# richardbaihe/a3t

Hardware: AMD Instinct MI355X
Metric: mel-frames/sec (train) (higher is better)
Workload: dtype bf16; 1 GPU; VCTK A3T masked-mel train step: 6+6 Conformer blocks d=384 H=2 ff=1536(k3), B=32/GPU, T_mel=1000, T_phn=120, postnet 5x256x5, fwd+bwd+clip+Adam, dropout 0.2/0.2/0.2 + postnet 0.5 (recipe); global_batch=32, parallelism=dp1, params=100799808

## Files before the change

a3t_amd/_lib.py:

```python
import ctypes
import os
from ctypes import POINTER, c_char_p, c_float, c_int, c_int32, c_int64, c_void_p

import torch

HERE = os.path.dirname(os.path.abspath(__file__))
LIB_PATH = os.environ.get("A3T_LIB_PATH") or os.path.join(HERE, "lib", "liba3t_hip.so")

F32, BF16 = 0, 1
ACT_NONE, ACT_RELU, ACT_TANH, ACT_SWISH = 0, 1, 2, 3
ACC_STORE, ACC_ADD, ACC_ATOMIC, ACC_SOLE = 0, 1, 2, 3


class GemmDesc(ctypes.Structure):
    _fields_ = [
        ("A", c_void_p), ("B", c_void_p), ("C", c_void_p), ("bias", c_void_p), ("R", c_void_p), ("S", c_void_p),
        ("M", c_int32), ("N", c_int32), ("K", c_int32),
        ("a_rs", c_int64), ("a_cs", c_int64),
        ("b_rs", c_int64), ("b_cs", c_int64), ("b_ts", c_int64),
        ("c_rs", c_int64),
        ("batch", c_int32), ("batch_inner", c_int32),
        ("a_bs0", c_int64), ("a_bs1", c_int64), ("b_bs0", c_int64), ("b_bs1", c_int64),
        ("c_bs0", c_int64), ("c_bs1", c_int64),
        ("taps", c_int32), ("pad", c_int32), ("dil", c_int32), ("Tseq", c_int32), ("kshift", c_int32),
# ... 41 lines not shown
    "a3t_mask_fill": [_P, _P, _P, _P, c_int, c_int, c_int, _P],
    "a3t_embed_finish_fwd": [_P, _P, _P, _P, _P, _P, _P, c_int, c_int, c_int, c_int, c_float, c_float, ctypes.c_uint32,
                             _P, _P],
    "a3t_embed_finish_bwd": [_P, _P, _P, _P, _P, _P, _P, _P, c_int, c_int, c_int, c_int, c_int, c_int, c_float, c_float,
                             ctypes.c_uint32, _P],
    "a3t_scale": [_P, _P, c_int64, c_float, _P],
    "a3t_axpy": [_P, _P, c_int64, c_float, _P],
    "a3t_attn_bias_fold": [_P, c_int32, c_int32, _P, _P, _P, _P],
    "a3t_scale_dev": [_P, _P, c_int64, _P, _P],
    "a3t_slice_rows": [_P, _P, c_int, c_int, c_int, c_int, c_int, c_int, _P],
    "a3t_concat_rows": [_P, _P, _P, c_int, c_int, c_int, c_int, _P],
    "a3t_concat_rows_ragged": [_P, _P, _P, _P, _P, c_int, c_int, c_int, c_int, c_int64, c_int64, _P],
    "a3t_split_rows": [_P, _P, _P, c_int, c_int, c_int, c_int, _P],
    "a3t_cast_bf16": [_P, _P, c_int64, _P],
    "a3t_cast_bf16_conv_t": [_P, _P, _P, _P, c_int, c_int, c_int, c_int, _P],
    "a3t_split_bf16": [_P, _P, _P, c_int64, _P],
    "a3t_reflect_pad": [_P, _P, c_int, c_int, c_int, c_int, _P],
    "a3t_reflect_pad_ragged": [_P, _P, _P, c_int, c_int, c_int, c_int, _P],
    "a3t_stft_amp": [_P, _P, c_int64, c_int, c_int, _P],
    "a3t_logmel_finish": [_P, _P, c_int, c_int, c_int, _P],
    "a3t_mlm_loss": [_P, _P, _P, _P, _P, _P, _P, _P, c_int, c_int, c_int, c_float, _P],
    "a3t_mlm_loss_scratch_floats": [c_int],
    "a3t_sumsq": [_P, c_int64, _P, _P],
    "a3t_clip_adam": [_P, _P, _P, _P, _P, _P, c_int64, c_float, c_float, c_float, c_float, c_int, c_float, c_float,
                      _P],
    "a3t_clip_adam_noam": [_P, _P, _P, _P, _P, _P, c_int64, _P, c_float, c_float, c_float, c_float, c_float, c_float,
                           c_float, c_float, _P],
    "a3t_sgd_step": [_P, _P, c_int64, c_float, c_float, _P],
    "a3t_pwg_gate": [_P, _P, _P, c_int64, c_int, _P],
    "a3t_pwg_res_skip": [_P, _P, _P, c_int64, c_int, c_int, _P],
    "a3t_pwg_upsample": [_P, _P, _P, c_int64, c_int64, c_int, c_int, _P],
    "a3t_replicate_pad": [_P, _P, c_int64, c_int64, c_int, c_int, _P],
    "a3t_bias_act": [_P, _P, c_int64, c_int, c_int, c_float, _P],
    "a3t_replicate_pad_ragged": [_P, _P, _P, c_int64, c_int64, c_int, c_int, _P],
    "a3t_pwg_upsample_ragged": [_P, _P, _P, _P, c_int, c_int64, c_int64, c_int, c_int, _P],
    "a3t_zero_tail": [_P, _P, c_int, c_int64, c_int64, c_int, _P],
    "a3t_layernorm_fwd_ragged": [_P, _P, _P, _P, _P, _P, _P, c_int, c_int, c_int, c_float, _P],
    "a3t_glu_dwconv_fwd_ragged": [_P, _P, _P, _P, _P, _P, c_int, c_int, c_int, c_int, _P],
    "a3t_relpos_softmax_fwd_ragged": [_P, _P, c_int, _P, _P, c_int, c_int, c_int, c_int, c_int64, c_int64, c_int64, c_float,
                                      _P],
    "a3t_splice_spans": [_P, _P, _P, _P, _P, _P, c_int, c_int, c_int, c_int, _P],
    "a3t_pwg_block_ragged": [_P, _P, _P, _P, _P, _P, _P, _P, _P, c_int, c_int, c_int, c_int, _P],
# ... 75 lines not shown
```

a3t_amd/conformer.py:

```python
import math
import os
import zlib
from dataclasses import dataclass

import torch

from . import ops
from ._lib import ACC_ADD, ACC_ATOMIC, ACC_STORE, ACT_RELU, ACT_SWISH, BF16, F32
from .config import A3TConfig
from .params import ParamStore
from .schedule import StepSchedule


def legacy_pe_table(c: A3TConfig) -> torch.Tensor:
    d = c.adim
    position = torch.arange(c.max_len - 1, -1, -1.0, dtype=torch.float32).unsqueeze(1)
    div = torch.exp(torch.arange(0, d, 2, dtype=torch.float32) * -(math.log(10000.0) / d))
    pe = torch.zeros(c.max_len, d)
    pe[:, 0::2] = torch.sin(position * div)
    pe[:, 1::2] = torch.cos(position * div)
    return pe


def score_chunks(lengths, heads, max_score_elems):
# ... 27 lines not shown
    ffn_keep4: bool = True
    lin_dgrad_t: bool = True
    fuse_ln_dropout: bool = True

    @classmethod
    def from_env(cls, environ=os.environ):
        fa, ft = environ.get("A3T_FUSED_ATTN", "auto"), environ.get("A3T_FUSED_ATTN_TRAIN", "1")
        if fa not in ("auto", "fwd", "0"):
            raise ValueError(f"A3T_FUSED_ATTN={fa!r}: expected auto, fwd or 0 (the flash backward behind '1' left the library in "
                             "round 5, tools/experiments/attn_flash_backward.patch)")
        on = {f: environ.get("A3T_" + f.upper(), "1") != "0" for f in
              ("side_stream", "side2", "wgrad_group", "post_f32_first", "attn_bwd_ds", "attn_signed", "attn_dq_dual",
               "attn_dbd_view", "attn_dk_main", "ffn_8p", "ffn_keep4", "lin_dgrad_t")}
        return cls(side_depth=max(2, int(environ.get("A3T_SIDE_DEPTH", "48"))), fused_attn=fa,
                   fused_attn_train=0 if ft == "0" else 2 if ft == "2" else 1, **on)


class ConformerStack(StepSchedule):
    def __init__(self, cfg: A3TConfig, store: ParamStore, compute: str = "f32", training: bool = True,
                 dropout: bool = False, options: EngineOptions = None):
        self.opt = opt = options if options is not None else EngineOptions.from_env()
        super().__init__(store.device, opt.side_stream, opt.side2, opt.side_depth)
        self.c = cfg
        self.dropping = bool(dropout and training)
        self.step_seed = 0
        self.store = store
        self.bf16 = (compute == "bf16")
        self.adt = torch.bfloat16 if self.bf16 else torch.float32
        self.cmp = BF16 if self.bf16 else F32
        self.training = training
# ... 13 lines not shown
        self._fused_now = self._fused_train_now = False
        self.attn_path, self.block_dims = {}, {}
        self._need_grad = training
        self._mode_tag = None
        if self.bf16:
            for n, v in (("adim", cfg.adim), ("ff", cfg.ff), ("idim", cfg.idim), ("odim", cfg.odim),
                         ("dk", cfg.dk), ("postnet_chans", cfg.postnet_chans or 8)):
                if v % 8:
                    raise ValueError(f"compute='bf16' needs {n} % 8 == 0 (16-byte DMA granules), got {v}")
            self.flat16 = torch.zeros(store.total, dtype=torch.bfloat16, device=self.dev)
            self.p16 = {k: self.flat16[o:o + math.prod(s)].view(s) for k, (o, s) in store.offsets.items()}
        self._ffn_plans = {}
        self._lin_plans = {}
        self._wt = {}
        self._P_ahead, self._pos_ev = {}, None
        self._cast_ev = self._wt_ev = None
        dec = [o for k, (o, _) in store.offsets.items() if k.startswith("dec.")]
        self._cast_split = min(dec) if dec else 0

    def _drop(self, p, tag):
        if not self.dropping or p <= 0.0:
            return None
        h = (zlib.crc32(tag.encode()) ^ ((self.step_seed * 0x9E3779B1) & 0xFFFFFFFF)) & 0xFFFFFFFF
        h = ((h ^ (h >> 16)) * 0x85EBCA6B) & 0xFFFFFFFF
        h = ((h ^ (h >> 13)) * 0xC2B2AE35) & 0xFFFFFFFF
        return (float(p), (h ^ (h >> 16)) & 0xFFFFFFFF)

    def _gm(self, g, tag, p, bias_grad, bias_scale):
        dr = self._drop(p, tag)
        if dr is None:
            return (self._g16(g) if self.bf16 else g)
        gm = self.ws.get(self._t("tmp.gm"), tuple(g.shape), self.adt)
        if self._gm_ready == tag:
            self._gm_ready = None
            return gm
        ops.dropout_bwd_cast(g, gm, dr[0], dr[1], colsum=bias_grad, colsum_scale=bias_scale)
        return gm

    def W(self, name):
        return self.p16[name] if self.bf16 else self.store.p[name]

    def refresh_weights(self):
        self._cast_ev = self._wt_ev = None
        if not self.bf16:
            return
        split = self._cast_split if self.side is not None else 0
        flat, flat16 = self.store.flat, self.flat16
        wt = list(self._wt.values()) if self._need_grad else []

        def transposed():
            for src_off, dst_off, _, tflat, shp in wt:
                ops.cast_bf16_conv_t(flat, tflat, src_off, dst_off, *shp)
        if split <= 0:
            ops.cast_bf16(flat, flat16)
            transposed()
            return
        ops.cast_bf16(flat[:split], flat16[:split])
        self._cast_ev = self._side(lambda: ops.cast_bf16(flat[split:], flat16[split:]), want_event="cast")
        if wt:
            self._wt_ev = self._side(transposed, want_event="wt")

    def _wait_cast(self, which):
        ev = getattr(self, which, None)
# ... 512 lines not shown
```

a3t_amd/csrc/misc.hip:

```cpp
#include <hip/hip_runtime.h>
#include <math.h>
#include <stdint.h>
#include "../../include/a3t_hip.h"
#include "dtype_io.h"

static inline int nblocks(int64_t n, int cap = 4096) {
    int64_t b = (n + 255) / 256;
    return (int)(b > cap ? cap : (b < 1 ? 1 : b));
}
#define GRID_STRIDE(i, n) \
    for (int64_t i = (int64_t)blockIdx.x * blockDim.x + threadIdx.x; i < (n); i += (int64_t)gridDim.x * blockDim.x)

__global__ void mask_fill_kernel(const float* __restrict__ x, const uint8_t* __restrict__ m,
                                 const float* __restrict__ mf, void* __restrict__ y, int y_dt, int64_t n, int C) {
    GRID_STRIDE(i, n) {
        int64_t r = i / C;
        int c = (int)(i - r * C);
        stx(y, y_dt, i, m[r] ? mf[c] : x[i]);
    }
}
extern "C" int a3t_mask_fill(const float* speech, const uint8_t* masked, const float* mask_feature, void* out,
                             int out_dtype, int M, int C, void* stream) {
    int64_t n = (int64_t)M * C;
    hipLaunchKernelGGL(mask_fill_kernel, dim3(nblocks(n)), dim3(256), 0, (hipStream_t)stream, speech, masked,
// ... 155 lines not shown
    }
    __syncthreads();
    for (int r = ty; r < 32; r += 8) {
        const int c = c0 + r, n = n0 + tx;
        if (c < C && n < N) Wt[((int64_t)c * taps + (taps - 1 - t)) * N + n] = io_f2bf(tile[tx][r]);
    }
}
extern "C" int a3t_cast_bf16_conv_t(const float* src, void* dst, const int64_t* src_off, const int64_t* dst_off, int count, int N,
                                    int taps, int C, void* stream) {
    if (count <= 0 || N <= 0 || taps <= 0 || C <= 0) return A3T_EINVAL;
    if (taps > 65535 || count > 65535) return A3T_EINVAL;
    dim3 grid((unsigned)(((N + 31) / 32) * ((C + 31) / 32)), (unsigned)taps, (unsigned)count);
    hipLaunchKernelGGL(cast_conv_t_kernel, grid, dim3(256), 0, (hipStream_t)stream, src, (unsigned short*)dst, src_off, dst_off, N, taps, C);
    return (int)hipGetLastError();
}
__global__ void split_bf16_kernel(const float* __restrict__ x, unsigned short* __restrict__ hi, unsigned short* __restrict__ lo,
                                  int64_t n4) {
    GRID_STRIDE(i, n4) {
        const float4 v = ((const float4*)x)[i];
        uint2 h, l;
        h.x = io_pack2(v.x, v.y);
        h.y = io_pack2(v.z, v.w);
        l.x = io_pack2(v.x - io_bf2f(h.x & 0xffff), v.y - io_bf2f(h.x >> 16));
        l.y = io_pack2(v.z - io_bf2f(h.y & 0xffff), v.w - io_bf2f(h.y >> 16));
        ((uint2*)hi)[i] = h;
        ((uint2*)lo)[i] = l;
    }
}
extern "C" int a3t_split_bf16(const float* x, void* hi, void* lo, int64_t n, void* stream) {
    if (n % 4 || ((uintptr_t)x & 15) || ((uintptr_t)hi & 7) || ((uintptr_t)lo & 7)) return A3T_EINVAL;
// ... 221 lines not shown
    red[threadIdx.x] = s;
    __syncthreads();
    for (int o = 128; o > 0; o >>= 1) {
        if (threadIdx.x < o) red[threadIdx.x] += red[threadIdx.x + o];
        __syncthreads();
    }
    if (threadIdx.x == 0) partial[blockIdx.x] = red[0];
}
__device__ __forceinline__ void adam_elem(float& p, const float g, float& m, float& v, const float coef, const float b1, const float b2,
                                          const float step_size, const float bc2s, const float eps) {
    const float gi = g * coef;
    m = m * b1 + (1.f - b1) * gi;
    v = v * b2 + (1.f - b2) * gi * gi;
    p -= step_size * m / (sqrtf(v) / bc2s + eps);
}
__device__ __forceinline__ void adam_sweep(float* __restrict__ p, const float* __restrict__ g, float* __restrict__ m, float* __restrict__ v,
                                           const int64_t n, const float coef, const float b1, const float b2, const float step_size,
                                           const float bc2s, const float eps) {
    const int64_t tid = (int64_t)blockIdx.x * blockDim.x + threadIdx.x, nthr = (int64_t)gridDim.x * blockDim.x;
    const bool vec = ((((uintptr_t)p) | ((uintptr_t)g) | ((uintptr_t)m) | ((uintptr_t)v)) & 15) == 0;
    const int64_t n4 = vec ? n / 4 : 0;
    for (int64_t i = tid; i < n4; i += nthr) {
        float4 pi = ((float4*)p)[i], mi = ((float4*)m)[i], vi = ((float4*)v)[i];
        const float4 gi = ((const float4*)g)[i];
        adam_elem(pi.x, gi.x, mi.x, vi.x, coef, b1, b2, step_size, bc2s, eps);
        adam_elem(pi.y, gi.y, mi.y, vi.y, coef, b1, b2, step_size, bc2s, eps);
        adam_elem(pi.z, gi.z, mi.z, vi.z, coef, b1, b2, step_size, bc2s, eps);
        adam_elem(pi.w, gi.w, mi.w, vi.w, coef, b1, b2, step_size, bc2s, eps);
        ((float4*)m)[i] = mi, ((float4*)v)[i] = vi, ((float4*)p)[i] = pi;
    }
    for (int64_t i = n4 * 4 + tid; i < n; i += nthr) adam_elem(p[i], g[i], m[i], v[i], coef, b1, b2, step_size, bc2s, eps);
}
extern "C" int a3t_sumsq(const float* g, int64_t n, double* partial, void* stream) {
    hipLaunchKernelGGL(sumsq_kernel, dim3(SUMSQ_BLOCKS), dim3(256), 0, (hipStream_t)stream, g, n, partial);
    return (int)hipGetLastError();
}
__global__ __launch_bounds__(256) void clip_adam_kernel(float* __restrict__ p, const float* __restrict__ g,
                                                        float* __restrict__ m, float* __restrict__ v,
                                                        const double* partial, float* norm_out, int64_t n, float lr,
                                                        float b1, float b2, float eps, float bc1, float bc2s,
                                                        float clip, float gscale) {
    __shared__ double red[256];
    double s = 0.0;
    for (int i = threadIdx.x; i < SUMSQ_BLOCKS; i += 256) s += partial[i];
    red[threadIdx.x] = s;
    __syncthreads();
// ... 7 lines not shown
    float coef = clip > 0.f ? clip / (norm + 1e-6f) : 1.f;
    coef = (coef > 1.f ? 1.f : coef) * gscale;
    const float step_size = lr / bc1;
    adam_sweep(p, g, m, v, n, coef, b1, b2, step_size, bc2s, eps);
}
extern "C" int a3t_clip_adam(float* p, const float* g, float* m, float* v, const double* partial, float* norm_out,
                             int64_t n, float lr, float beta1, float beta2, float eps, int step, float clip,
                             float gscale, void* stream) {
    const float bc1 = (float)(1.0 - pow((double)beta1, (double)step));
    const float bc2s = (float)sqrt(1.0 - pow((double)beta2, (double)step));
    hipLaunchKernelGGL(clip_adam_kernel, dim3(nblocks(n / 4, 2048)), dim3(256), 0, (hipStream_t)stream, p, g, m, v, partial,
                       norm_out, n, lr, beta1, beta2, eps, bc1, bc2s, clip, gscale);
    return (int)hipGetLastError();
}

__global__ __launch_bounds__(256) void clip_adam_noam_kernel(float* __restrict__ p, const float* __restrict__ g,
                                                             float* __restrict__ m, float* __restrict__ v,
                                                             const double* partial, float* norm_out, int64_t n,
                                                             const int* state, float base_lr, float model_size,
                                                             float warmup, float b1, float b2, float eps, float clip,
                                                             float gscale) {
    __shared__ double red[256];
    double s = 0.0;
    for (int i = threadIdx.x; i < SUMSQ_BLOCKS; i += 256) s += partial[i];
    red[threadIdx.x] = s;
    __syncthreads();
    for (int o = 128; o > 0; o >>= 1) {
        if (threadIdx.x < o) red[threadIdx.x] += red[threadIdx.x + o];
        __syncthreads();
    }
    const float norm = (float)sqrt(red[0]) * fabsf(gscale);
    if (blockIdx.x == 0 && threadIdx.x == 0) norm_out[0] = norm;
    if (!isfinite(norm)) return;
    const double t = (double)(state[0] + 1);
    const float lr = (float)((double)base_lr * pow((double)model_size, -0.5) * fmin(pow(t, -0.5), t * pow((double)warmup, -1.5)));
    const float bc1 = (float)(1.0 - pow((double)b1, t));
    const float bc2s = (float)sqrt(1.0 - pow((double)b2, t));
    float coef = clip > 0.f ? clip / (norm + 1e-6f) : 1.f;
    coef = (coef > 1.f ? 1.f : coef) * gscale;
    const float step_size = lr / bc1;
    adam_sweep(p, g, m, v, n, coef, b1, b2, step_size, bc2s, eps);
}
__global__ void adam_state_advance_kernel(const float* norm, int* state) {
    if (isfinite(norm[0])) state[0] += 1; else state[1] += 1;
}
extern "C" int a3t_clip_adam_noam(float* p, const float* g, float* m, float* v, const double* partial, float* norm_out,
                                  int64_t n, int* state, float base_lr, float model_size, float warmup, float beta1,
                                  float beta2, float eps, float clip, float gscale, void* stream) {
    hipLaunchKernelGGL(clip_adam_noam_kernel, dim3(nblocks(n / 4, 2048)), dim3(256), 0, (hipStream_t)stream, p, g, m, v,
                       partial, norm_out, n, state, base_lr, model_size, warmup, beta1, beta2, eps, clip, gscale);
    hipLaunchKernelGGL(adam_state_advance_kernel, dim3(1), dim3(1), 0, (hipStream_t)stream, norm_out, state);
    return (int)hipGetLastError();
}

__global__ __launch_bounds__(256) void sgd_step_kernel(float* __restrict__ p, const float* __restrict__ g, const int64_t n,
                                                       const float step) {
    const int64_t tid = (int64_t)blockIdx.x * blockDim.x + threadIdx.x, nthr = (int64_t)gridDim.x * blockDim.x;
    const bool vec = ((((uintptr_t)p) | ((uintptr_t)g)) & 15) == 0;
    const int64_t n4 = vec ? n / 4 : 0;
    for (int64_t i = tid; i < n4; i += nthr) {
        float4 pi = ((float4*)p)[i];
        const float4 gi = ((const float4*)g)[i];
        pi.x -= step * gi.x, pi.y -= step * gi.y, pi.z -= step * gi.z, pi.w -= step * gi.w;
        ((float4*)p)[i] = pi;
    }
// ... 281 lines not shown
```

a3t_amd/engine.py:

```python
import math
from typing import Dict

import torch

from . import ops
from ._lib import ACT_NONE, ACT_TANH, F32
from .conformer import ConformerStack, score_chunks


class MLMEngine(ConformerStack):
    def _begin(self, batch, need_grad):
        speech = batch["speech"].contiguous()
        B, Tm, idim = speech.shape
        text = batch["text"].contiguous()
        Tp = text.shape[1]
        self.dims = (B, Tm, Tp, Tm + Tp)
        self.attn_path, self.block_dims = {}, {}
        self._need_grad = bool(need_grad)
        self._mode_tag = ops.gemm_mode_tag()
        self.step_seed += 1
        self.refresh_weights()
        self._arena_clear("fwd64")
        self._P_ahead, self._pos_ev = {}, None
        return speech.view(B * Tm, idim), text, batch["masked_position"].contiguous().view(torch.uint8)

    def _prologue(self, batch, speech2, text, masked, split):
        c, p, ws = self.c, self.store.p, self.ws
        B, Tm, Tp, T = self.dims
        d, pp = c.adim, c.positional_dropout_rate
        spos = batch["speech_segment_pos"].contiguous()
        tpos = batch["text_segment_pos"].contiguous()
        xm = self._act("emb.xm", (B * Tm, c.idim))
        ops.mask_fill(speech2, masked, p["mask_feature"], xm)
        e0 = ws.get("emb.e0", (B * Tm, d))
        ops.linear_fwd(xm, self.W("emb.w"), e0, bias=p["emb.b"], compute=self.cmp)
        e = self._ln_fwd("emb.ln", e0, "emb.ln", eps=1e-5, out_dtype=torch.float32)
# ... 65 lines not shown
            y = o
        after = ws.get("head.after", (B * Tm, c.odim))
        after.copy_(before)
        ops.axpy(y, after, 1.0)
        return hs, before, after

    def forward(self, batch: Dict[str, torch.Tensor], need_grad: bool = True, gscale: float = 1.0, lens=None):
        if lens is not None:
            return self._forward_rows_alone(batch, need_grad, lens)
        c, ws = self.c, self.ws
        (B, Tm, _), Tp, d = batch["speech"].shape, batch["text"].shape[1], c.adim
        T = Tm + Tp
        if self.bf16 and (T % 8 or Tm % 8):
            raise ValueError(f"compute='bf16' needs T_mel and T_mel+T_phn to be multiples of 8, got {Tm}, {T}")
        self._fused_now, self._fused_train_now = main_path = self._attn_choice(B, T, need_grad)
        speech2, text, masked = self._begin(batch, need_grad)
        pp = c.positional_dropout_rate
        keymask = ws.get("keymask", (B, T), torch.uint8)
        keymask[:, :Tm].copy_(batch["speech_mask"].reshape(B, Tm).view(torch.uint8))
        keymask[:, Tm:].copy_(batch["text_mask"].reshape(B, Tp).view(torch.uint8))
        xs, xsp, xst = self._prologue(batch, speech2, text, masked, split=c.pre_blocks > 0)
        pos_e = self._act("pos.enc", (T, d))
        pos_d = self._act("pos.dec", (T, d))
        pos_on_side = None
        if self._drop(pp, "pos.enc"):
            def drop_pos():
                pf = ws.get("pos.f32", (T, d))
                pf[:Tm].copy_(self.pe[:Tm])
                pf[Tm:].copy_(self.pe[:Tp])
                ops.dropout(pf, pos_e, *self._drop(pp, "pos.enc"))
                pf.copy_(self.pe[:T])
# ... 15 lines not shown
                def run():
                    if kind == first and pos_on_side is not None:
                        pos_on_side()
                    for i in range(n):
                        tag = f"{kind}.{i}.mha"
                        P = self._act(tag + ".P", (posx.shape[0], d))
                        ops.linear_fwd(posx, self.W(tag + ".wpos"), P, compute=self.cmp)
                        self._P_ahead[tag] = P
                return run
            self._pos_ev = {}
            if c.pre_blocks > 0:
                self._pos_ev["pre"] = self._side(project("pre", pos_e[:Tm], c.pre_blocks), want_event="pos.pre")
            self._pos_ev["enc"] = self._side(project("enc", pos_e, c.enc_blocks), want_event="pos.enc")
            if c.has_decoder:
                self._pos_ev["dec"] = self._side(project("dec", pos_d, c.dec_blocks), want_event="pos.dec")
        if c.pre_blocks > 0:
            kms = ws.get("keymask.pre", (B, Tm), torch.uint8)
            kms.copy_(batch["speech_mask"].reshape(B, Tm).view(torch.uint8))
            self._fused_now, self._fused_train_now = self._attn_choice(B, Tm, need_grad)
            x = xsp
            for i in range(c.pre_blocks):
                x = self.block_fwd(f"pre.{i}", x, pos_e[:Tm], kms, B, Tm)
            self._fused_now, self._fused_train_now = main_path
            xs = ws.get("emb.xs", (B * T, d))
            ops.concat_rows(x, xst, xs, B, Tm, Tp, d)
        x = self._encode(xs, B, T, (pos_e, keymask), (pos_d, keymask), self._drop(pp, "dec.x"))
        hs, before, after = self._head(x)
        loss = ws.get("head.loss", (1,))
        scratch = ws.get("head.lscratch", (ops.loss_scratch_floats(B * Tm),))
        db = ws.get("head.dbefore", (B * Tm, c.odim)) if need_grad else None
# ... 154 lines not shown
```

a3t_amd/ops.py:

```python
import ctypes
import os

import torch

from . import _lib as L
from ._lib import ACC_ADD, ACC_ATOMIC, ACC_SOLE, ACC_STORE, ACT_NONE, ACT_RELU, ACT_SWISH, ACT_TANH, BF16, F32

__all__ = ["gemm", "gemm_plan", "linear_fwd", "linear_bwd_data", "linear_bwd_weight", "conv_fwd", "conv_bwd_data",
           "conv_bwd_weight"]


PROFILE = None


def _stream():
    return ctypes.c_void_p(torch.cuda.current_stream().cuda_stream)


def _ptr(t):
    if t is None:
        return None
    return ctypes.c_void_p(t.data_ptr())


# ... 379 lines not shown


def attn_bias_fold(slots, S, d, gu, gv, gbqkv):
    L.check(L.load().a3t_attn_bias_fold(_ptr(slots), S, d, _ptr(gu), _ptr(gv), _ptr(gbqkv), _stream()), "attn_bias_fold")


def cast_bf16(x, y):
    L.check(L.load().a3t_cast_bf16(_ptr(x), _ptr(y), x.numel(), _stream()), "cast_bf16")


def cast_bf16_conv_t(src_flat, dst, src_off, dst_off, N, taps, C):
    L.check(L.load().a3t_cast_bf16_conv_t(_ptr(src_flat), _ptr(dst), _ptr(src_off), _ptr(dst_off), src_off.numel(), N, taps, C,
                                          _stream()), "cast_bf16_conv_t")


def split_bf16(x, hi, lo):
    L.check(L.load().a3t_split_bf16(_ptr(x), _ptr(hi), _ptr(lo), x.numel(), _stream()), "split_bf16")


def slice_rows(x, y, B, T, Tm, D, reverse_add=False):
    L.check(L.load().a3t_slice_rows(_ptr(x), _ptr(y), _dt(y), B, T, Tm, D, int(reverse_add), _stream()), "slice_rows")


def concat_rows(speech, text, xs, B, Tm, Tp, D):
    L.check(L.load().a3t_concat_rows(_ptr(speech), _ptr(text), _ptr(xs), B, Tm, Tp, D, _stream()), "concat_rows")


def concat_rows_ragged(speech, text, xs, slens, tlens, B, Tm, Tp, D, speech_bs=None, text_bs=None):
    L.check(L.load().a3t_concat_rows_ragged(_ptr(speech), _ptr(text), _ptr(xs), _ptr(_i32(slens, "slens")),
                                            _ptr(_i32(tlens, "tlens")), B, Tm, Tp, D, Tm * D if speech_bs is None else speech_bs,
# ... 42 lines not shown

def sumsq(g, partial):
    L.check(L.load().a3t_sumsq(_ptr(g), g.numel(), _ptr(partial), _stream()), "sumsq")


def clip_adam(p, g, m, v, partial, norm_out, lr, step, clip=1.0, gscale=1.0, betas=(0.9, 0.999), eps=1e-8):
    L.check(L.load().a3t_clip_adam(_ptr(p), _ptr(g), _ptr(m), _ptr(v), _ptr(partial), _ptr(norm_out), p.numel(), lr,
                                   betas[0], betas[1], eps, step, clip, gscale, _stream()), "clip_adam")


def clip_adam_noam(p, g, m, v, partial, norm_out, state, base_lr, model_size, warmup, clip=1.0, gscale=1.0,
                   betas=(0.9, 0.999), eps=1e-8):
    L.check(L.load().a3t_clip_adam_noam(_ptr(p), _ptr(g), _ptr(m), _ptr(v), _ptr(partial), _ptr(norm_out), p.numel(),
                                        _ptr(state), base_lr, float(model_size), float(warmup), betas[0], betas[1], eps,
                                        clip, gscale, _stream()), "clip_adam_noam")


def sgd_step(p, g, lr, gscale=1.0):
    if p.dtype != torch.float32 or g.dtype != torch.float32 or p.numel() != g.numel() or not (p.is_contiguous() and g.is_contiguous()):
        raise ValueError("sgd_step: p and g must be contiguous fp32 buffers of one size")
    L.check(L.load().a3t_sgd_step(_ptr(p), _ptr(g), p.numel(), float(lr), float(gscale), _stream()), "sgd_step")


def pwg_gate(y, c, out):
    T, H = out.shape
    L.check(L.load().a3t_pwg_gate(_ptr(y), _ptr(c), _ptr(out), T, H, _stream()), "pwg_gate")


def pwg_res_skip(o, x, skips):
    T, R = x.shape
# ... 417 lines not shown
```

a3t_amd/trainer.py:

```python
import os
from typing import Dict, List, Sequence

import torch
import torch.distributed as dist

from .config import A3TConfig


def shard_batches(batches: Sequence[Sequence[str]], rank: int, world: int) -> List[List[str]]:
    for b in batches:
        if len(b) < world:
            raise RuntimeError(f"The batch-size must be equal or more than world_size: {len(b)} < {world}")
    return [list(b[rank::world]) for b in batches]


def noam_lr(step: int, base_lr: float, model_size: int, warmup: int) -> float:
    return base_lr * model_size ** -0.5 * min(step ** -0.5, step * warmup ** -1.5)


def iterator_stop(local_done: bool, device="cpu") -> bool:
    if not (dist.is_available() and dist.is_initialized()):
        return local_done
    t = torch.tensor([1 if local_done else 0], dtype=torch.int64, device=device)
    dist.all_reduce(t, op=dist.ReduceOp.SUM)
# ... 70 lines not shown
                with torch.cuda.stream(self.stream):
                    w.wait()
                    self.g[rng[0]:rng[1]].copy_(self.stage[rng[0]:rng[1]])
            else:
                w.wait()
                self.g[rng[0]:rng[1]].copy_(self.stage[rng[0]:rng[1]])
        self.works = []
        if self.cuda:
            torch.cuda.current_stream().wait_stream(self.stream)


class A3TTrainer:

    def __init__(self, cfg: A3TConfig, store, compute="bf16", lr=1.0, warmup_steps=4000, grad_clip=1.0,
                 betas=(0.9, 0.999), eps=1e-8, overlap=True, dropout=True, force_reducer=False,
                 bucket_min_elems=16 * 1024 * 1024, comm_dtype=torch.float32):
        from .engine import MLMEngine
        self.cfg, self.store = cfg, store
        self.engine = MLMEngine(cfg, store, compute=compute, training=True, dropout=dropout)
        dev = store.device
        self.m = torch.zeros_like(store.flat)
        self.v = torch.zeros_like(store.flat)
        self.partial = torch.zeros(1024, dtype=torch.float64, device=dev)
        self.norm = torch.zeros(1, device=dev)
        self.step_no = 0
        self.opt_state = torch.zeros(2, dtype=torch.int32, device=dev)
        self.comm_dtype = comm_dtype
        self.lr, self.warmup, self.clip, self.betas, self.eps = lr, warmup_steps, grad_clip, betas, eps
        self.world = dist.get_world_size() if (dist.is_available() and dist.is_initialized()) else 1
        self._main = None
        if dev.type == "cuda":
            from .schedule import shared_stream
            self._main = shared_stream(dev, "main", high=True)
        self.reducer = None
# ... 33 lines not shown
        w = 1.0
        if total_weight is not None:
            w = grad_scale(float(batch["speech"].shape[0]), float(total_weight), self.world)
        out = self.engine.forward(batch, gscale=w / accum_grad)
        last = (accum_index == accum_grad - 1)
        if self.reducer is not None and last:
            self._backward_overlapped()
        else:
            self.engine.backward()
            if self.world > 1 and last:
                dist.all_reduce(st.grad)
        if not last:
            return out["loss"]
        self.step_no += 1
        ops.sumsq(st.grad, self.partial)
        ops.clip_adam_noam(st.flat, st.grad, self.m, self.v, self.partial, self.norm, self.opt_state, self.lr,
                           self.cfg.adim, self.warmup, clip=self.clip, gscale=1.0 / self.world, betas=self.betas,
                           eps=self.eps)
        return out["loss"]

    def optimizer_steps(self):
        a, sk = self.opt_state.tolist()
        if sk:
            import logging
            logging.warning(f"{sk} step(s) had a non-finite gradient norm and were skipped (trainer.py:640-645)")
        return a, sk

    def _backward_overlapped(self):
        eng, red = self.engine, self.reducer
        state = {"next": 0}
        lows = [lo for lo, _ in red.ranges]
        offs = self.store.offsets

# ... 28 lines not shown
```

include/a3t_hip.h:

```cpp
#ifndef A3T_HIP_H
#define A3T_HIP_H
#include <stdint.h>

#ifdef __cplusplus
extern "C" {
#endif

#define A3T_F32 0
#define A3T_BF16 1

#define A3T_EINVAL (-22)

#define A3T_ACT_NONE 0
#define A3T_ACT_RELU 1
#define A3T_ACT_TANH 2
#define A3T_ACT_SWISH 3

#define A3T_ACC_STORE 0
#define A3T_ACC_ADD 1
#define A3T_ACC_ATOMIC 2
#define A3T_ACC_SOLE 3

typedef struct a3t_gemm_desc {
    const void* A;
// ... 101 lines not shown
                         const int64_t* tpos, float* de, float* demb, float* dseg, int B, int Tm, int Tp,
                         int D, int V, int nseg, float xscale, float drop_p, uint32_t drop_key, void* stream);
int a3t_scale(const float* x, float* y, int64_t n, float s, void* stream);
int a3t_axpy(const float* x, float* y, int64_t n, float a, void* stream);
int a3t_attn_bias_fold(const float* slots, int S, int d, float* gu, float* gv, float* gbqkv, void* stream);
int a3t_scale_dev(const float* x, float* y, int64_t n, const float* s, void* stream);
int a3t_slice_rows(const float* x, void* y, int y_dtype, int B, int T, int Tm, int D, int reverse_add,
                   void* stream);
int a3t_concat_rows(const float* speech, const float* text, float* xs, int B, int Tm, int Tp, int D, void* stream);
int a3t_split_rows(const float* dxs, float* dspeech, float* dtext, int B, int Tm, int Tp, int D, void* stream);
int a3t_concat_rows_ragged(const float* speech, const float* text, float* xs, const int32_t* slens, const int32_t* tlens, int B,
                           int Tm, int Tp, int D, int64_t speech_bs, int64_t text_bs, void* stream);
int a3t_cast_bf16(const float* x, void* y, int64_t n, void* stream);
int a3t_cast_bf16_conv_t(const float* src, void* dst, const int64_t* src_off, const int64_t* dst_off, int count, int N,
                         int taps, int C, void* stream);
int a3t_split_bf16(const float* x, void* hi, void* lo, int64_t n, void* stream);

int a3t_reflect_pad(const float* x, float* out, int B, int N, int pad, int ld, void* stream);
int a3t_reflect_pad_ragged(const float* x, float* out, const int32_t* lens, int B, int N, int pad, int ld, void* stream);
int a3t_stft_amp(const float* S, float* amp, int64_t rows, int nbins, int ld, void* stream);
int a3t_logmel_finish(float* mel, const int64_t* olens, int B, int F, int C, void* stream);

int a3t_mlm_loss(const float* before, const float* after, const float* target, const uint8_t* masked,
                 float* loss_out, float* d_before, float* d_after, float* scratch, int M, int C, int l2,
                 float gscale, void* stream);
int a3t_mlm_loss_scratch_floats(int M);

int a3t_sumsq(const float* g, int64_t n, double* partial , void* stream);
int a3t_clip_adam(float* p, const float* g, float* m, float* v, const double* partial, float* norm_out,
                  int64_t n, float lr, float beta1, float beta2, float eps, int step, float clip,
                  float gscale, void* stream);

int a3t_clip_adam_noam(float* p, const float* g, float* m, float* v, const double* partial, float* norm_out, int64_t n,
                       int32_t* state, float base_lr, float model_size, float warmup, float beta1, float beta2,
                       float eps, float clip, float gscale, void* stream);

int a3t_sgd_step(float* p, const float* g, int64_t n, float lr, float gscale, void* stream);

int a3t_pwg_gate(const float* y, const float* c, float* out, int64_t T, int H, void* stream);
int a3t_pwg_res_skip(const float* o, float* x, float* skips, int64_t T, int R, int S, void* stream);
int a3t_pwg_upsample(const float* c, const float* w, float* out, int64_t B, int64_t Tin, int C, int scale,
                     void* stream);
int a3t_replicate_pad(const float* x, float* y, int64_t B, int64_t T, int C, int pad, void* stream);
int a3t_bias_act(float* x, const float* bias, int64_t M, int C, int act, float scale, void* stream);
int a3t_replicate_pad_ragged(const float* x, float* y, const int32_t* lens, int64_t B, int64_t T, int C, int pad,
                             void* stream);
int a3t_pwg_upsample_ragged(const float* c, const float* w, float* out, const int32_t* lens, int mul, int64_t B,
                            int64_t Tin, int C, int scale, void* stream);
int a3t_zero_tail(float* x, const int32_t* lens, int mul, int64_t B, int64_t T, int C, void* stream);
int a3t_layernorm_fwd_ragged(const float* x, const float* gamma, const float* beta, float* y, float* mean, float* rstd,
// ... 90 lines not shown
```

Before: 825,700 mel-frames/s.

## Fuse bf16 weight shadow write into Adam and transpose conv weights from bf16

The Adam kernel now also writes the bf16 copy of the updated parameters, so the next step can skip the separate fp32-to-bf16 cast pass over all ~100M parameters when a version stamp shows the image is fresh. Transposed conv weights are then built from the bf16 image with a single batched tiled-transpose kernel driven by a device table, and this launch is deferred until after the positional projections are queued on the side stream. This removes a full read of the fp32 parameters and many small launches per step. In exchange it adds extra bf16 writes inside Adam, staleness tracking through tensor versions, and a fallback path when alignment fails.

```diff
diff --git a/a3t_amd/_lib.py b/a3t_amd/_lib.py
--- a/a3t_amd/_lib.py
+++ b/a3t_amd/_lib.py
@@ -79,6 +79,7 @@
     "a3t_split_rows": [_P, _P, _P, c_int, c_int, c_int, c_int, _P],
     "a3t_cast_bf16": [_P, _P, c_int64, _P],
     "a3t_cast_bf16_conv_t": [_P, _P, _P, _P, c_int, c_int, c_int, c_int, _P],
+    "a3t_cast_bf16_conv_t_from16": [_P, _P, _P, _P, c_int, _P],
     "a3t_split_bf16": [_P, _P, _P, c_int64, _P],
     "a3t_reflect_pad": [_P, _P, c_int, c_int, c_int, c_int, _P],
     "a3t_reflect_pad_ragged": [_P, _P, _P, c_int, c_int, c_int, c_int, _P],
@@ -91,6 +92,8 @@
                       _P],
     "a3t_clip_adam_noam": [_P, _P, _P, _P, _P, _P, c_int64, _P, c_float, c_float, c_float, c_float, c_float, c_float,
                            c_float, c_float, _P],
+    "a3t_clip_adam_noam_shadow": [_P, _P, _P, _P, _P, _P, c_int64, _P, c_float, c_float, c_float, c_float, c_float, c_float,
+                                  c_float, c_float, _P, _P],
     "a3t_sgd_step": [_P, _P, c_int64, c_float, c_float, _P],
     "a3t_pwg_gate": [_P, _P, _P, c_int64, c_int, _P],
     "a3t_pwg_res_skip": [_P, _P, _P, c_int64, c_int, c_int, _P],
diff --git a/a3t_amd/conformer.py b/a3t_amd/conformer.py
--- a/a3t_amd/conformer.py
+++ b/a3t_amd/conformer.py
@@ -65,6 +65,10 @@
                "attn_dbd_view", "attn_dk_main", "ffn_8p", "ffn_keep4", "lin_dgrad_t")}
         return cls(side_depth=max(2, int(environ.get("A3T_SIDE_DEPTH", "48"))), fused_attn=fa,
                    fused_attn_train=0 if ft == "0" else 2 if ft == "2" else 1, **on)
+
+
+def image_fresh(stamp, flat, flat16, bf16=True):
+    return bool(bf16) and stamp is not None and stamp[0] == flat._version and stamp[1] is flat16
 
 
 class ConformerStack(StepSchedule):
@@ -108,7 +112,9 @@
         self._lin_plans = {}
         self._wt = {}
         self._P_ahead, self._pos_ev = {}, None
-        self._cast_ev = self._wt_ev = None
+        self._cast_ev = self._wt_ev = self._wt_deferred = None
+        self._wt_tab = None
+        self.image_stamp, self.image_source = None, None
         dec = [o for k, (o, _) in store.offsets.items() if k.startswith("dec.")]
         self._cast_split = min(dec) if dec else 0
 
@@ -134,13 +140,47 @@
     def W(self, name):
         return self.p16[name] if self.bf16 else self.store.p[name]
 
-    def refresh_weights(self):
-        self._cast_ev = self._wt_ev = None
+    def _wt_table(self):
+        key = tuple((suf, w[3].data_ptr()) for suf, w in self._wt.items())
+        if self._wt_tab is None or self._wt_tab[0] != key:
+            base = next(iter(self._wt.values()))[3]
+            rows = []
+            for src_off, dst_off, _, tflat, shp in self._wt.values():
+                rel = tflat.data_ptr() - base.data_ptr()
+                rows += [(s, rel // 2 + d, *shp) for s, d in zip(src_off.tolist(), dst_off.tolist())]
+            ok = base.data_ptr() % 16 == 0 and self.flat16.data_ptr() % 16 == 0 and \
+                all(v % 8 == 0 for r in rows for v in (r[0], r[1], r[2], r[4]))
+            self._wt_tab = (key, (base, ops.conv_t_table(rows, self.dev)) if ok else None)
+        return self._wt_tab[1]
+
+    def flush_wt(self):
+        run, self._wt_deferred = self._wt_deferred, None
+        if run is not None:
+            self._wt_ev = self._side(run, want_event="wt")
+
+    def refresh_weights(self, defer_wt=False):
+        self._cast_ev = self._wt_ev = self._wt_deferred = None
         if not self.bf16:
             return
         split = self._cast_split if self.side is not None else 0
         flat, flat16 = self.store.flat, self.flat16
         wt = list(self._wt.values()) if self._need_grad else []
+        if image_fresh(self.image_stamp, flat, flat16):
+            self.image_source = "adam"
+            table = self._wt_table() if wt else None
+            if wt and table is None:
+                def run():
+                    for src_off, dst_off, _, tflat, shp in wt:
+                        ops.cast_bf16_conv_t(flat, tflat, src_off, dst_off, *shp)
+            elif wt:
+                def run():
+                    ops.cast_bf16_conv_t_from16(flat16, table[0], table[1])
+            if wt:
+                self._wt_deferred = run
+                if not defer_wt:
+                    self.flush_wt()
+            return
+        self.image_source, self.image_stamp = "cast", None
 
         def transposed():
             for src_off, dst_off, _, tflat, shp in wt:
diff --git a/a3t_amd/csrc/misc.hip b/a3t_amd/csrc/misc.hip
--- a/a3t_amd/csrc/misc.hip
+++ b/a3t_amd/csrc/misc.hip
@@ -193,6 +193,61 @@
     hipLaunchKernelGGL(cast_conv_t_kernel, grid, dim3(256), 0, (hipStream_t)stream, src, (unsigned short*)dst, src_off, dst_off, N, taps, C);
     return (int)hipGetLastError();
 }
+#define CT16_TILE 64
+#define CT16_PITCH 33
+__global__ __launch_bounds__(256) void cast_conv_t_from16_kernel(const unsigned short* __restrict__ src, unsigned short* __restrict__ dst,
+                                                                const int64_t* __restrict__ table) {
+    __shared__ unsigned int tile[CT16_TILE * CT16_PITCH];
+    const int64_t* e = table + 5 * (int64_t)blockIdx.y;
+    const int N = (int)e[2], taps = (int)e[3], C = (int)e[4];
+    const int tn = (N + CT16_TILE - 1) / CT16_TILE, tc = (C + CT16_TILE - 1) / CT16_TILE;
+    if (blockIdx.x >= (unsigned)(tn * tc * taps)) return;
+    const unsigned short* W = src + e[0];
+    unsigned short* Wt = dst + e[1];
+    const int t = blockIdx.x / (tn * tc), r = blockIdx.x - t * (tn * tc);
+    const int n0 = (r / tc) * CT16_TILE, c0 = (r % tc) * CT16_TILE;
+    for (int q = threadIdx.x; q < CT16_TILE * 8; q += 256) {
+        const int row = q >> 3, j = q & 7;
+        const int n = n0 + row, c = c0 + 8 * j;
+        uint4 v = make_uint4(0u, 0u, 0u, 0u);
+        if (n < N && c < C) v = *(const uint4*)(W + ((int64_t)n * taps + t) * C + c);
+        unsigned int* d = tile + row * CT16_PITCH + 4 * j;
+        d[0] = v.x, d[1] = v.y, d[2] = v.z, d[3] = v.w;
+    }
+    __syncthreads();
+    const unsigned short* th = (const unsigned short*)tile;
+    for (int q = threadIdx.x; q < CT16_TILE * 8; q += 256) {
+        const int row = q >> 3, j = q & 7;
+        const int c = c0 + row, n = n0 + 8 * j;
+        if (c >= C || n >= N) continue;
+        unsigned int o[4];
+#pragma unroll
+        for (int k = 0; k < 4; ++k) {
+            const unsigned int lo = th[(8 * j + 2 * k) * (2 * CT16_PITCH) + row];
+            const unsigned int hi = th[(8 * j + 2 * k + 1) * (2 * CT16_PITCH) + row];
+            o[k] = lo | (hi << 16);
+        }
+        *(uint4*)(Wt + ((int64_t)c * taps + (taps - 1 - t)) * N + n) = make_uint4(o[0], o[1], o[2], o[3]);
+    }
+}
+extern "C" int a3t_cast_bf16_conv_t_from16(const void* src16, void* dst, const int64_t* table_host, const int64_t* table_dev,
+                                           int count, void* stream) {
+    if (!src16 || !dst || !table_host || !table_dev || count <= 0 || count > 65535) return A3T_EINVAL;
+    if (((uintptr_t)src16 | (uintptr_t)dst) & 15) return A3T_EINVAL;
+    int64_t tiles = 0;
+    for (int i = 0; i < count; ++i) {
+        const int64_t* e = table_host + 5 * (int64_t)i;
+        const int64_t N = e[2], taps = e[3], C = e[4];
+        if (N <= 0 || taps <= 0 || C <= 0 || N > INT32_MAX || taps > 65535 || C > INT32_MAX) return A3T_EINVAL;
+        if ((N | C | e[0] | e[1]) & 7) return A3T_EINVAL;
+        const int64_t k = ((N + CT16_TILE - 1) / CT16_TILE) * ((C + CT16_TILE - 1) / CT16_TILE) * taps;
+        if (k > INT32_MAX) return A3T_EINVAL;
+        tiles = k > tiles ? k : tiles;
+    }
+    hipLaunchKernelGGL(cast_conv_t_from16_kernel, dim3((unsigned)tiles, (unsigned)count), dim3(256), 0, (hipStream_t)stream,
+                       (const unsigned short*)src16, (unsigned short*)dst, table_dev);
+    return (int)hipGetLastError();
+}
 __global__ void split_bf16_kernel(const float* __restrict__ x, unsigned short* __restrict__ hi, unsigned short* __restrict__ lo,
                                   int64_t n4) {
     GRID_STRIDE(i, n4) {
@@ -444,11 +499,12 @@
     v = v * b2 + (1.f - b2) * gi * gi;
     p -= step_size * m / (sqrtf(v) / bc2s + eps);
 }
+template <bool SHADOW = false>
 __device__ __forceinline__ void adam_sweep(float* __restrict__ p, const float* __restrict__ g, float* __restrict__ m, float* __restrict__ v,
                                            const int64_t n, const float coef, const float b1, const float b2, const float step_size,
-                                           const float bc2s, const float eps) {
+                                           const float bc2s, const float eps, unsigned short* __restrict__ w16 = nullptr) {
     const int64_t tid = (int64_t)blockIdx.x * blockDim.x + threadIdx.x, nthr = (int64_t)gridDim.x * blockDim.x;
-    const bool vec = ((((uintptr_t)p) | ((uintptr_t)g) | ((uintptr_t)m) | ((uintptr_t)v)) & 15) == 0;
+    const bool vec = ((((uintptr_t)p) | ((uintptr_t)g) | ((uintptr_t)m) | ((uintptr_t)v) | (SHADOW ? 2 * (uintptr_t)w16 : 0)) & 15) == 0;
     const int64_t n4 = vec ? n / 4 : 0;
     for (int64_t i = tid; i < n4; i += nthr) {
         float4 pi = ((float4*)p)[i], mi = ((float4*)m)[i], vi = ((float4*)v)[i];
@@ -458,8 +514,21 @@
         adam_elem(pi.z, gi.z, mi.z, vi.z, coef, b1, b2, step_size, bc2s, eps);
         adam_elem(pi.w, gi.w, mi.w, vi.w, coef, b1, b2, step_size, bc2s, eps);
         ((float4*)m)[i] = mi, ((float4*)v)[i] = vi, ((float4*)p)[i] = pi;
-    }
-    for (int64_t i = n4 * 4 + tid; i < n; i += nthr) adam_elem(p[i], g[i], m[i], v[i], coef, b1, b2, step_size, bc2s, eps);
+        if (SHADOW) ((uint2*)w16)[i] = make_uint2(io_pack2(pi.x, pi.y), io_pack2(pi.z, pi.w));
+    }
+    for (int64_t i = n4 * 4 + tid; i < n; i += nthr) {
+        adam_elem(p[i], g[i], m[i], v[i], coef, b1, b2, step_size, bc2s, eps);
+        if (SHADOW) w16[i] = io_f2bf(p[i]);
+    }
+}
+__device__ __forceinline__ void shadow_sweep(const float* __restrict__ p, unsigned short* __restrict__ w16, const int64_t n) {
+    const int64_t tid = (int64_t)blockIdx.x * blockDim.x + threadIdx.x, nthr = (int64_t)gridDim.x * blockDim.x;
+    const int64_t n4 = (((uintptr_t)p | 2 * (uintptr_t)w16) & 15) == 0 ? n / 4 : 0;
+    for (int64_t i = tid; i < n4; i += nthr) {
+        const float4 pi = ((const float4*)p)[i];
+        ((uint2*)w16)[i] = make_uint2(io_pack2(pi.x, pi.y), io_pack2(pi.z, pi.w));
+    }
+    for (int64_t i = n4 * 4 + tid; i < n; i += nthr) w16[i] = io_f2bf(p[i]);
 }
 extern "C" int a3t_sumsq(const float* g, int64_t n, double* partial, void* stream) {
     hipLaunchKernelGGL(sumsq_kernel, dim3(SUMSQ_BLOCKS), dim3(256), 0, (hipStream_t)stream, g, n, partial);
@@ -497,12 +566,13 @@
     return (int)hipGetLastError();
 }
 
+template <bool SHADOW>
 __global__ __launch_bounds__(256) void clip_adam_noam_kernel(float* __restrict__ p, const float* __restrict__ g,
                                                              float* __restrict__ m, float* __restrict__ v,
                                                              const double* partial, float* norm_out, int64_t n,
                                                              const int* state, float base_lr, float model_size,
                                                              float warmup, float b1, float b2, float eps, float clip,
-                                                             float gscale) {
+                                                             float gscale, unsigned short* __restrict__ w16) {
     __shared__ double red[256];
     double s = 0.0;
     for (int i = threadIdx.x; i < SUMSQ_BLOCKS; i += 256) s += partial[i];
@@ -514,7 +584,10 @@
     }
     const float norm = (float)sqrt(red[0]) * fabsf(gscale);
     if (blockIdx.x == 0 && threadIdx.x == 0) norm_out[0] = norm;
-    if (!isfinite(norm)) return;
+    if (!isfinite(norm)) {
+        if (SHADOW) shadow_sweep(p, w16, n);
+        return;
+    }
     const double t = (double)(state[0] + 1);
     const float lr = (float)((double)base_lr * pow((double)model_size, -0.5) * fmin(pow(t, -0.5), t * pow((double)warmup, -1.5)));
     const float bc1 = (float)(1.0 - pow((double)b1, t));
@@ -522,7 +595,7 @@
     float coef = clip > 0.f ? clip / (norm + 1e-6f) : 1.f;
     coef = (coef > 1.f ? 1.f : coef) * gscale;
     const float step_size = lr / bc1;
-    adam_sweep(p, g, m, v, n, coef, b1, b2, step_size, bc2s, eps);
+    adam_sweep<SHADOW>(p, g, m, v, n, coef, b1, b2, step_size, bc2s, eps, w16);
 }
 __global__ void adam_state_advance_kernel(const float* norm, int* state) {
     if (isfinite(norm[0])) state[0] += 1; else state[1] += 1;
@@ -530,8 +603,19 @@
 extern "C" int a3t_clip_adam_noam(float* p, const float* g, float* m, float* v, const double* partial, float* norm_out,
                                   int64_t n, int* state, float base_lr, float model_size, float warmup, float beta1,
                                   float beta2, float eps, float clip, float gscale, void* stream) {
-    hipLaunchKernelGGL(clip_adam_noam_kernel, dim3(nblocks(n / 4, 2048)), dim3(256), 0, (hipStream_t)stream, p, g, m, v,
-                       partial, norm_out, n, state, base_lr, model_size, warmup, beta1, beta2, eps, clip, gscale);
+    hipLaunchKernelGGL(clip_adam_noam_kernel<false>, dim3(nblocks(n / 4, 2048)), dim3(256), 0, (hipStream_t)stream, p, g, m, v,
+                       partial, norm_out, n, state, base_lr, model_size, warmup, beta1, beta2, eps, clip, gscale,
+                       (unsigned short*)nullptr);
+    hipLaunchKernelGGL(adam_state_advance_kernel, dim3(1), dim3(1), 0, (hipStream_t)stream, norm_out, state);
+    return (int)hipGetLastError();
+}
+extern "C" int a3t_clip_adam_noam_shadow(float* p, const float* g, float* m, float* v, const double* partial, float* norm_out,
+                                         int64_t n, int* state, float base_lr, float model_size, float warmup, float beta1,
+                                         float beta2, float eps, float clip, float gscale, void* w_bf16, void* stream) {
+    if (!w_bf16 || ((uintptr_t)w_bf16 & 1)) return A3T_EINVAL;
+    hipLaunchKernelGGL(clip_adam_noam_kernel<true>, dim3(nblocks(n / 4, 2048)), dim3(256), 0, (hipStream_t)stream, p, g, m, v,
+                       partial, norm_out, n, state, base_lr, model_size, warmup, beta1, beta2, eps, clip, gscale,
+                       (unsigned short*)w_bf16);
     hipLaunchKernelGGL(adam_state_advance_kernel, dim3(1), dim3(1), 0, (hipStream_t)stream, norm_out, state);
     return (int)hipGetLastError();
 }
diff --git a/a3t_amd/engine.py b/a3t_amd/engine.py
--- a/a3t_amd/engine.py
+++ b/a3t_amd/engine.py
@@ -9,7 +9,7 @@
 
 
 class MLMEngine(ConformerStack):
-    def _begin(self, batch, need_grad):
+    def _begin(self, batch, need_grad, defer_wt=False):
         speech = batch["speech"].contiguous()
         B, Tm, idim = speech.shape
         text = batch["text"].contiguous()
@@ -19,7 +19,7 @@
         self._need_grad = bool(need_grad)
         self._mode_tag = ops.gemm_mode_tag()
         self.step_seed += 1
-        self.refresh_weights()
+        self.refresh_weights(defer_wt=defer_wt)
         self._arena_clear("fwd64")
         self._P_ahead, self._pos_ev = {}, None
         return speech.view(B * Tm, idim), text, batch["masked_position"].contiguous().view(torch.uint8)
@@ -115,7 +115,7 @@
         if self.bf16 and (T % 8 or Tm % 8):
             raise ValueError(f"compute='bf16' needs T_mel and T_mel+T_phn to be multiples of 8, got {Tm}, {T}")
         self._fused_now, self._fused_train_now = main_path = self._attn_choice(B, T, need_grad)
-        speech2, text, masked = self._begin(batch, need_grad)
+        speech2, text, masked = self._begin(batch, need_grad, defer_wt=True)
         pp = c.positional_dropout_rate
         keymask = ws.get("keymask", (B, T), torch.uint8)
         keymask[:, :Tm].copy_(batch["speech_mask"].reshape(B, Tm).view(torch.uint8))
@@ -161,6 +161,7 @@
             self._pos_ev["enc"] = self._side(project("enc", pos_e, c.enc_blocks), want_event="pos.enc")
             if c.has_decoder:
                 self._pos_ev["dec"] = self._side(project("dec", pos_d, c.dec_blocks), want_event="pos.dec")
+        self.flush_wt()
         if c.pre_blocks > 0:
             kms = ws.get("keymask.pre", (B, Tm), torch.uint8)
             kms.copy_(batch["speech_mask"].reshape(B, Tm).view(torch.uint8))
diff --git a/a3t_amd/ops.py b/a3t_amd/ops.py
--- a/a3t_amd/ops.py
+++ b/a3t_amd/ops.py
@@ -417,6 +417,17 @@
                                           _stream()), "cast_bf16_conv_t")
 
 
+def conv_t_table(entries, device):
+    host = torch.tensor([list(e) for e in entries], dtype=torch.int64).reshape(-1, 5).contiguous()
+    return host, host.to(device)
+
+
+def cast_bf16_conv_t_from16(src16, dst, table):
+    host, dev = table
+    L.check(L.load().a3t_cast_bf16_conv_t_from16(_ptr(src16), _ptr(dst), ctypes.c_void_p(host.data_ptr()), _ptr(dev),
+                                                 host.shape[0], _stream()), "cast_bf16_conv_t_from16")
+
+
 def split_bf16(x, hi, lo):
     L.check(L.load().a3t_split_bf16(_ptr(x), _ptr(hi), _ptr(lo), x.numel(), _stream()), "split_bf16")
 
@@ -489,6 +500,15 @@
     L.check(L.load().a3t_clip_adam_noam(_ptr(p), _ptr(g), _ptr(m), _ptr(v), _ptr(partial), _ptr(norm_out), p.numel(),
                                         _ptr(state), base_lr, float(model_size), float(warmup), betas[0], betas[1], eps,
                                         clip, gscale, _stream()), "clip_adam_noam")
+
+
+def clip_adam_noam_shadow(p, g, m, v, partial, norm_out, state, base_lr, model_size, warmup, w16, clip=1.0, gscale=1.0,
+                          betas=(0.9, 0.999), eps=1e-8):
+    if w16.dtype != torch.bfloat16 or w16.numel() != p.numel() or not w16.is_contiguous():
+        raise ValueError("clip_adam_noam_shadow: w16 must be a contiguous bf16 buffer of p's size")
+    L.check(L.load().a3t_clip_adam_noam_shadow(_ptr(p), _ptr(g), _ptr(m), _ptr(v), _ptr(partial), _ptr(norm_out), p.numel(),
+                                               _ptr(state), base_lr, float(model_size), float(warmup), betas[0], betas[1],
+                                               eps, clip, gscale, _ptr(w16), _stream()), "clip_adam_noam_shadow")
 
 
 def sgd_step(p, g, lr, gscale=1.0):
diff --git a/a3t_amd/trainer.py b/a3t_amd/trainer.py
--- a/a3t_amd/trainer.py
+++ b/a3t_amd/trainer.py
@@ -108,10 +108,11 @@
 
     def __init__(self, cfg: A3TConfig, store, compute="bf16", lr=1.0, warmup_steps=4000, grad_clip=1.0,
                  betas=(0.9, 0.999), eps=1e-8, overlap=True, dropout=True, force_reducer=False,
-                 bucket_min_elems=16 * 1024 * 1024, comm_dtype=torch.float32):
+                 bucket_min_elems=16 * 1024 * 1024, comm_dtype=torch.float32, adam_shadow=None):
         from .engine import MLMEngine
         self.cfg, self.store = cfg, store
         self.engine = MLMEngine(cfg, store, compute=compute, training=True, dropout=dropout)
+        self.adam_shadow = (os.environ.get("A3T_ADAM_SHADOW", "1") != "0") if adam_shadow is None else bool(adam_shadow)
         dev = store.device
         self.m = torch.zeros_like(store.flat)
         self.v = torch.zeros_like(store.flat)
@@ -175,9 +176,16 @@
             return out["loss"]
         self.step_no += 1
         ops.sumsq(st.grad, self.partial)
-        ops.clip_adam_noam(st.flat, st.grad, self.m, self.v, self.partial, self.norm, self.opt_state, self.lr,
-                           self.cfg.adim, self.warmup, clip=self.clip, gscale=1.0 / self.world, betas=self.betas,
-                           eps=self.eps)
+        eng = self.engine
+        kw = dict(clip=self.clip, gscale=1.0 / self.world, betas=self.betas, eps=self.eps)
+        if self.adam_shadow and eng.bf16 and getattr(eng, "flat16", None) is not None:
+            ops.clip_adam_noam_shadow(st.flat, st.grad, self.m, self.v, self.partial, self.norm, self.opt_state, self.lr,
+                                      self.cfg.adim, self.warmup, eng.flat16, **kw)
+            eng.image_stamp = (st.flat._version, eng.flat16)
+        else:
+            ops.clip_adam_noam(st.flat, st.grad, self.m, self.v, self.partial, self.norm, self.opt_state, self.lr,
+                               self.cfg.adim, self.warmup, **kw)
+            eng.image_stamp = None
         return out["loss"]
 
     def optimizer_steps(self):
diff --git a/include/a3t_hip.h b/include/a3t_hip.h
--- a/include/a3t_hip.h
+++ b/include/a3t_hip.h
@@ -139,6 +139,8 @@
 int a3t_cast_bf16(const float* x, void* y, int64_t n, void* stream);
 int a3t_cast_bf16_conv_t(const float* src, void* dst, const int64_t* src_off, const int64_t* dst_off, int count, int N,
                          int taps, int C, void* stream);
+int a3t_cast_bf16_conv_t_from16(const void* src16, void* dst, const int64_t* table_host, const int64_t* table_dev, int count,
+                                void* stream);
 int a3t_split_bf16(const float* x, void* hi, void* lo, int64_t n, void* stream);
 
 int a3t_reflect_pad(const float* x, float* out, int B, int N, int pad, int ld, void* stream);
@@ -159,6 +161,9 @@
 int a3t_clip_adam_noam(float* p, const float* g, float* m, float* v, const double* partial, float* norm_out, int64_t n,
                        int32_t* state, float base_lr, float model_size, float warmup, float beta1, float beta2,
                        float eps, float clip, float gscale, void* stream);
+int a3t_clip_adam_noam_shadow(float* p, const float* g, float* m, float* v, const double* partial, float* norm_out, int64_t n,
+                              int32_t* state, float base_lr, float model_size, float warmup, float beta1, float beta2,
+                              float eps, float clip, float gscale, void* w_bf16, void* stream);
 
 int a3t_sgd_step(float* p, const float* g, int64_t n, float lr, float gscale, void* stream);
 
```

Result: no change. 829,800 mel-frames/s (median of 6 runs) (+0.5%).
